# raulmur/ORB_SLAM2

Hardware: NVIDIA H100
Metric: stereo frames/sec (ORB extract L+R + ComputeStereoMatches, KITTI-shaped 1242x375 @2000 kpts) (higher is better)
Workload: dtype u8

## Files before the change

### orb_slam2_b200/csrc/borb_host.cu

```cuda
#include <cmath>
#include <cstdarg>
#include <cstdio>
#include <algorithm>
#include <cstdlib>
#include <cstring>

#include "borb_internal.h"

namespace borb {

static thread_local std::string tl_error;
void set_error(const char* fmt, ...) {
    char buf[512];
    va_list ap;
    va_start(ap, fmt);
    vsnprintf(buf, sizeof(buf), fmt, ap);
    va_end(ap);
    tl_error = buf;
}

bool allow_max_smem(const void* func) {
    static std::mutex mu;
    static std::vector<std::pair<const void*, int>> done;
    int dev = 0;
// ... 123 lines not shown
        v.hCell = (int)std::ceil(height / v.nRows);
        v.pitch = align_up(v.w + 8, 128);
        v.pyr_off = pyr_off;
        pyr_off += (unsigned)v.pitch * v.h;
        v.cellsPerBlk = FAST_TILE_W / v.wCell > 0 ? FAST_TILE_W / v.wCell : 1;
        v.blkCols = (v.nCols + v.cellsPerBlk - 1) / v.cellsPerBlk;
        v.blkBase = blk;
        blk += v.blkCols * v.nRows;
        v.cand_off = cand_off;
        v.cand_cap = v.nCols * v.nRows * ((v.wCell + 1) / 2) * ((v.hCell + 1) / 2);
        cand_off += (unsigned)align_up(v.cand_cap, 32);
        v.quota = e->per_level[l];
        v.nIni = (int)std::round(width / height);
        if (v.nIni < 1) { set_error("level %d aspect ratio gives zero quadtree roots (reference divides by zero)", l); return BORB_ERR_UNSUPPORTED; }
        v.hX = width / v.nIni;
        v.node_cap = (v.quota > 4 * v.nIni ? v.quota : 4 * v.nIni) + 3;
        v.node_cap = align_up(v.node_cap + 1, 4);
        v.sel_off = sel_off;
        sel_off += v.node_cap;
        v.scale = e->scale[l];
        v.inv_scale = e->inv_scale[l];
        v.patch_size = (float)(int)(PATCH * e->scale[l]);
        g.blur_base[l] = btile;
        btile += ((v.w + BLUR_TILE_W - 1) / BLUR_TILE_W) * ((v.h + BLUR_TILE_H - 1) / BLUR_TILE_H);
        if (l > 0) {
            const int wpad = (v.w + 8 + 3) & ~3;
            v.xtab_off = (unsigned)(tabs.size() / 4);
            resize_table(g.lv[l - 1].w, v.w, true, wpad - v.w, tabs);
            v.ytab_off = (unsigned)(tabs.size() / 4);
            resize_table(g.lv[l - 1].h, v.h, false, 0, tabs);
            v.xwin_off = (unsigned)(tabs.size() / 4);
            std::vector<int16_t> win;
            v.x_windowed = resize_window_table(tabs, (size_t)v.xtab_off * 4, wpad, win) ? 1 : 0;
            tabs.insert(tabs.end(), win.begin(), win.end());
        }
        if (quadtree_smem_bytes(v.node_cap) > 200 * 1024) {
            set_error("per-level quota %d exceeds the quadtree kernel's shared-memory envelope", v.quota);
            return BORB_ERR_UNSUPPORTED;
        }
    }
    g.blur_base[L] = btile;
    g.blur_tiles = btile;
    g.fast_blocks = blk;
    g.pyr_image_stride = (unsigned)align_up((int)pyr_off, g.lv[0].pitch);
    g.cand_image_stride = cand_off;
    g.sel_image_stride = sel_off;
    if (sel_off >= 65536) { set_error("keypoint capacity %d exceeds 65535", sel_off); return BORB_ERR_UNSUPPORTED; }
// ... 75 lines not shown
    cudaEventRecord(e->ev[(size_t)e->ev_slot * 9 + i], e->stream);
    e->ev_mask[e->ev_slot] |= 1u << i;
}
void drain_timing(borb_extractor* e) {
    const int R = borb_extractor::EV_RING;
    for (int k = e->ev_pending - 1; k >= 0; k--) {
        const int slot = ((e->ev_slot - k) % R + R) % R;
        const unsigned m = e->ev_mask[slot];
        for (int i = 0; i < 8; i++) {
            float ms = 0.f;
            if (m & (1u << i)) {
                int j = i + 1;
                while (j < 9 && !(m & (1u << j))) j++;
                if (j < 9 && cudaEventElapsedTime(&ms, e->ev[(size_t)slot * 9 + i], e->ev[(size_t)slot * 9 + j]) != cudaSuccess) { ms = 0.f; cudaGetLastError(); }
            }
            e->stage_ms[i] = ms;
            e->stage_sum_ms[i] += ms;
        }
        e->stage_steps++;
    }
    e->ev_pending = 0;
}

borb_status enqueue_extract(borb_extractor* e, int n) {
    const Geometry& g = e->geom;
    Workspace& ws = e->ws;
    cudaStream_t s = e->stream;
    BORB_CUDA(cudaMemsetAsync(ws.cand_cnt, 0, (size_t)n * g.nlevels * sizeof(int), s));
    mark(e, 1);
    e->launches += launch_pyramid(g, ws, n, s);
    mark(e, 2);
    e->launches += launch_fast(g, ws, n, s);
    mark(e, 3);
    e->launches += launch_quadtree(g, ws, n, s);
    mark(e, 4);
    e->launches += launch_blur(g, ws, n, s);
    mark(e, 5);
    e->launches += launch_describe(g, ws, n, s);
    mark(e, 6);
    BORB_CUDA(cudaGetLastError());
    e->last_n_images = n;
    e->last_stereo_pairs = 0;
    return BORB_OK;
}

borb_status rectified_size(borb_extractor* e, int w, int h, int* gw, int* gh) {
    if (!e->d_map[0][0]) return BORB_OK;
    if (w != e->map_src_w || h != e->map_src_h) {
        set_error("rectification maps were built for %dx%d raw frames, got %dx%d", e->map_src_w, e->map_src_h, w, h);
        return BORB_ERR_INVALID_ARG;
    }
    *gw = e->map_dst_w; *gh = e->map_dst_h;
    return BORB_OK;
}

borb_status upload_slots(borb_extractor* e, const uint8_t* const* slots, int n, int w, int h, int stride, bool stereo_pairs = false) {
    const Geometry& g = e->geom;
    const int ch = e->in_channels;
    if (stride < w * ch) { set_error("stride %d smaller than a row of %d %d-channel pixels", stride, w, ch); return BORB_ERR_INVALID_ARG; }
    const size_t img_bytes = (size_t)stride * h;
    bool contiguous = n > 1 || ch > 1 || e->d_map[0][0] != nullptr;
    for (int k = 0; k < n; k++) {
        if (!slots[k]) { set_error("image %d is NULL", k); return BORB_ERR_INVALID_ARG; }
        if (slots[k] != slots[0] + (size_t)k * img_bytes) contiguous = false;
    }
    auto need_stage = [&](size_t need) -> borb_status {
        if (e->ws.stage_bytes < need) {
            BORB_CUDA(cudaStreamSynchronize(e->stream));
            cudaFree(e->ws.stage);
            e->ws.stage = nullptr; e->ws.stage_bytes = 0;
            BORB_CUDA(cudaMalloc(&e->ws.stage, need));
            e->ws.stage_bytes = need;
        }
        return BORB_OK;
    };
    if (e->d_map[0][0]) {
        if (ch != 1) { set_error("rectification maps apply to CV_8UC1 frames"); return BORB_ERR_UNSUPPORTED; }
        const size_t src_img = contiguous ? img_bytes : (size_t)w * h;
        const int src_stride = contiguous ? stride : w;
        borb_status st = need_stage(src_img * n);
        if (st != BORB_OK) return st;
        if (contiguous) BORB_CUDA(cudaMemcpyAsync(e->ws.stage, slots[0], src_img * n, cudaMemcpyHostToDevice, e->stream));
        else
            for (int k = 0; k < n; k++)
                BORB_CUDA(cudaMemcpy2DAsync(e->ws.stage + (size_t)k * src_img, w, slots[k], stride, w, h, cudaMemcpyHostToDevice, e->stream));
        e->launches += launch_repack_remap(g, e->ws, e->ws.stage, src_stride, src_img, w, h, e->d_map[0][0], e->d_map[0][1],
                                           stereo_pairs ? e->d_map[1][0] : nullptr, stereo_pairs ? e->d_map[1][1] : nullptr, n, e->stream);
        return BORB_OK;
    }
    if (contiguous) {
        const size_t need = img_bytes * n;
        borb_status st = need_stage(need);
        if (st != BORB_OK) return st;
        BORB_CUDA(cudaMemcpyAsync(e->ws.stage, slots[0], need, cudaMemcpyHostToDevice, e->stream));
        if (ch == 1) e->launches += launch_repack(g, e->ws, e->ws.stage, stride, img_bytes, n, e->stream);
        else e->launches += launch_repack_color(g, e->ws, e->ws.stage, stride, img_bytes, ch, e->in_rgb, n, e->stream);
        return BORB_OK;
    }
    if (ch > 1) {
        const size_t row = (size_t)w * ch;
        borb_status st = need_stage(row * h * n);
        if (st != BORB_OK) return st;
        for (int k = 0; k < n; k++)
            BORB_CUDA(cudaMemcpy2DAsync(e->ws.stage + (size_t)k * row * h, row, slots[k], stride, row, h, cudaMemcpyHostToDevice, e->stream));
        e->launches += launch_repack_color(g, e->ws, e->ws.stage, (int)row, row * h, ch, e->in_rgb, n, e->stream);
        return BORB_OK;
    }
    for (int k = 0; k < n; k++) {
        uint8_t* dst = e->ws.pyr + (size_t)k * g.pyr_image_stride + g.lv[0].pyr_off;
        BORB_CUDA(cudaMemcpy2DAsync(dst, g.lv[0].pitch, slots[k], stride, w, h, cudaMemcpyHostToDevice, e->stream));
    }
    return BORB_OK;
}

borb_status upload_device(borb_extractor* e, const uint8_t* d_gray, int n, int w, int h, size_t pitch, size_t image_stride) {
    const Geometry& g = e->geom;
    cudaMemcpy3DParms p = {};
    p.srcPtr = make_cudaPitchedPtr((void*)d_gray, pitch, w, image_stride / pitch);
    p.dstPtr = make_cudaPitchedPtr(e->ws.pyr + g.lv[0].pyr_off, g.lv[0].pitch, w, g.pyr_image_stride / g.lv[0].pitch);
    if (image_stride % pitch == 0 && g.pyr_image_stride % g.lv[0].pitch == 0) {
        p.extent = make_cudaExtent(w, h, n);
        p.kind = cudaMemcpyDeviceToDevice;
        BORB_CUDA(cudaMemcpy3DAsync(&p, e->stream));
    } else {
        for (int i = 0; i < n; i++)
            BORB_CUDA(cudaMemcpy2DAsync(e->ws.pyr + (size_t)i * g.pyr_image_stride + g.lv[0].pyr_off, g.lv[0].pitch,
                                        d_gray + (size_t)i * image_stride, pitch, w, h, cudaMemcpyDeviceToDevice, e->stream));
    }
    return BORB_OK;
}

borb_status download_kps(borb_extractor* e, int first, int count, int step, borb_keypoint* kps, uint8_t* desc, int cap, int* n_out) {
    const Geometry& g = e->geom;
    const int m = cap < g.sel_image_stride ? cap : g.sel_image_stride;
    cudaStream_t s = e->stream;
    if (kps && m > 0)
        BORB_CUDA(cudaMemcpy2DAsync(kps, (size_t)cap * sizeof(borb_keypoint), e->ws.kps + (size_t)first * g.sel_image_stride,
                                    (size_t)step * g.sel_image_stride * sizeof(borb_keypoint), (size_t)m * sizeof(borb_keypoint),
                                    count, cudaMemcpyDeviceToHost, s));
    if (desc && m > 0)
        BORB_CUDA(cudaMemcpy2DAsync(desc, (size_t)cap * 32, e->ws.desc + (size_t)first * g.sel_image_stride * 32,
                                    (size_t)step * g.sel_image_stride * 32, (size_t)m * 32, count, cudaMemcpyDeviceToHost, s));
    if (n_out)
        BORB_CUDA(cudaMemcpy2DAsync(n_out, sizeof(int), e->ws.nkp + first, (size_t)step * sizeof(int), sizeof(int), count,
                                    cudaMemcpyDeviceToHost, s));
    return BORB_OK;
}

borb_status check_args(borb_extractor* e, int n, int w, int h) {
    if (!e) { set_error("null handle"); return BORB_ERR_INVALID_ARG; }
// ... 157 lines not shown
borb_status borb_extractor_reserve(borb_extractor* e, int width, int height, int max_images) {
    if (!e || max_images < 1) return BORB_ERR_INVALID_ARG;
    return ensure(e, width, height, max_images);
}

borb_status borb_sync(borb_extractor* e) {
    if (!e) return BORB_ERR_INVALID_ARG;
    BORB_CUDA(cudaSetDevice(e->device));
    BORB_CUDA(cudaStreamSynchronize(e->stream));
    return finish_timing(e);
}

borb_status borb_extract_batch_enqueue(borb_extractor* e, const uint8_t* const* gray, int n, int w, int h, int stride,
                                       borb_keypoint* kps, uint8_t* desc, int cap, int* n_out) {
    borb_status st = check_args(e, n, w, h);
    if (st != BORB_OK) return st;
    if (n == 0) return BORB_OK;
    if (!gray || cap < 0 || stride < w) { set_error("bad arguments"); return BORB_ERR_INVALID_ARG; }
    int gw = w, gh = h;
    if ((st = rectified_size(e, w, h, &gw, &gh)) != BORB_OK) return st;
    if ((st = ensure(e, gw, gh, n)) != BORB_OK) return st;
    begin_step(e);
    mark(e, 0);
    if ((st = upload_slots(e, gray, n, w, h, stride)) != BORB_OK) return st;
    if ((st = enqueue_extract(e, n)) != BORB_OK) return st;
    mark(e, 7);
    st = download_kps(e, 0, n, 1, kps, desc, cap, n_out);
    mark(e, 8);
    return st;
}

borb_status borb_extract_batch(borb_extractor* e, const uint8_t* const* gray, int n, int w, int h, int stride,
                               borb_keypoint* kps, uint8_t* desc, int cap, int* n_out) {
    if (!n_out) { set_error("n_out is required"); return BORB_ERR_INVALID_ARG; }
    borb_status st = borb_extract_batch_enqueue(e, gray, n, w, h, stride, kps, desc, cap, n_out);
    if (st != BORB_OK) return st;
    if (n == 0) return BORB_OK;
    if ((st = borb_sync(e)) != BORB_OK) return st;
    for (int i = 0; i < n; i++)
        if (n_out[i] > cap) { set_error("image %d produced %d keypoints, capacity %d", i, n_out[i], cap); return BORB_ERR_CAPACITY; }
    return BORB_OK;
}

borb_status borb_extract(borb_extractor* e, const uint8_t* gray, int w, int h, int stride, borb_keypoint* kps, uint8_t* desc,
                         int cap, int* n_out) {
    if (!n_out) { set_error("n_out is required"); return BORB_ERR_INVALID_ARG; }
    *n_out = 0;
    if (!gray || w == 0 || h == 0) return BORB_OK;
    const uint8_t* one[1] = {gray};
    return borb_extract_batch(e, one, 1, w, h, stride, kps, desc, cap, n_out);
}

borb_status borb_extract_batch_device(borb_extractor* e, const uint8_t* d_gray, int n, int w, int h, size_t pitch,
                                      size_t image_stride, borb_keypoint* kps, uint8_t* desc, int cap, int* n_out) {
    borb_status st = check_args(e, n, w, h);
    if (st != BORB_OK) return st;
    if (n == 0) return BORB_OK;
    if (!d_gray || pitch < (size_t)w) { set_error("bad arguments"); return BORB_ERR_INVALID_ARG; }
    if ((st = ensure(e, w, h, n)) != BORB_OK) return st;
    begin_step(e);
    mark(e, 0);
    if ((st = upload_device(e, d_gray, n, w, h, pitch, image_stride)) != BORB_OK) return st;
    if ((st = enqueue_extract(e, n)) != BORB_OK) return st;
    mark(e, 7);
    if ((st = download_kps(e, 0, n, 1, kps, desc, cap, n_out)) != BORB_OK) return st;
    mark(e, 8);
    return borb_sync(e);
}

borb_status borb_extractor_set_rectify_maps(borb_extractor* e, int which, const float* map_x, const float* map_y, int src_w, int src_h,
                                            int dst_w, int dst_h) {
    if (!e || which < 0 || which > 1) { set_error("bad arguments"); return BORB_ERR_INVALID_ARG; }
    BORB_CUDA(cudaSetDevice(e->device));
    BORB_CUDA(cudaStreamSynchronize(e->stream));
    if (!map_x || !map_y) {
        for (int s2 = which; s2 < 2; s2++)
            for (int c = 0; c < 2; c++) { cudaFree(e->d_map[s2][c]); e->d_map[s2][c] = nullptr; }
        return BORB_OK;
    }
    if (src_w <= 0 || src_h <= 0 || dst_w <= 0 || dst_h <= 0) { set_error("bad map geometry"); return BORB_ERR_INVALID_ARG; }
    if (which == 1 && (!e->d_map[0][0] || src_w != e->map_src_w || src_h != e->map_src_h || dst_w != e->map_dst_w || dst_h != e->map_dst_h)) {
        set_error("install the left maps (set 0) first; both sets share one geometry"); return BORB_ERR_STATE;
    }
    const size_t bytes = (size_t)dst_w * dst_h * sizeof(float);
    const float* src[2] = {map_x, map_y};
    for (int c = 0; c < 2; c++) {
// ... 138 lines not shown
    BORB_CUDA(cudaSetDevice(left->device));
    BORB_CUDA(cudaStreamSynchronize(right->stream));
    begin_step(left);
    borb_status st = enqueue_stereo(left, right, 1, nullptr, nullptr, bf, b);
    if (st != BORB_OK) return st;
    if ((st = download_stereo(left, 1, u_right, depth, cap)) != BORB_OK) return st;
    mark(left, 8);
    return borb_sync(left);
}

borb_status borb_stereo_frames_enqueue(borb_extractor* e, const uint8_t* const* left, const uint8_t* const* right, int n_pairs,
                                       int w, int h, int stride, float bf, float b, borb_keypoint* kps_left, uint8_t* desc_left,
                                       int* n_left, borb_keypoint* kps_right, uint8_t* desc_right, int* n_right, float* u_right,
                                       float* depth, int cap) {
    borb_status st = check_args(e, n_pairs, w, h);
    if (st != BORB_OK) return st;
    if (n_pairs == 0) return BORB_OK;
    if (!left || !right || stride < w || !(b > 0.f)) { set_error("bad arguments"); return BORB_ERR_INVALID_ARG; }
    int gw = w, gh = h;
    if ((st = rectified_size(e, w, h, &gw, &gh)) != BORB_OK) return st;
    if ((st = ensure(e, gw, gh, 2 * n_pairs)) != BORB_OK) return st;
    begin_step(e);
    mark(e, 0);
    {
        std::vector<const uint8_t*> slots(2 * (size_t)n_pairs);
        for (int p = 0; p < n_pairs; p++) { slots[2 * p] = left[p]; slots[2 * p + 1] = right[p]; }
        if ((st = upload_slots(e, slots.data(), 2 * n_pairs, w, h, stride, true)) != BORB_OK) return st;
    }
    if ((st = enqueue_extract(e, 2 * n_pairs)) != BORB_OK) return st;
    if ((st = enqueue_stereo(e, e, n_pairs, nullptr, nullptr, bf, b)) != BORB_OK) return st;
    if ((st = download_kps(e, 0, n_pairs, 2, kps_left, desc_left, cap, n_left)) != BORB_OK) return st;
    if ((st = download_kps(e, 1, n_pairs, 2, kps_right, desc_right, cap, n_right)) != BORB_OK) return st;
    if ((st = download_stereo(e, n_pairs, u_right, depth, cap)) != BORB_OK) return st;
    mark(e, 8);
    return BORB_OK;
}

borb_status borb_stereo_frames(borb_extractor* e, const uint8_t* const* left, const uint8_t* const* right, int n_pairs, int w,
                               int h, int stride, float bf, float b, borb_keypoint* kps_left, uint8_t* desc_left, int* n_left,
                               borb_keypoint* kps_right, uint8_t* desc_right, int* n_right, float* u_right, float* depth, int cap) {
    borb_status st = borb_stereo_frames_enqueue(e, left, right, n_pairs, w, h, stride, bf, b, kps_left, desc_left, n_left,
                                                kps_right, desc_right, n_right, u_right, depth, cap);
    if (st != BORB_OK || n_pairs == 0) return st;
    if ((st = borb_sync(e)) != BORB_OK) return st;
    for (int p = 0; p < n_pairs; p++)
        if ((n_left && n_left[p] > cap) || (n_right && n_right[p] > cap)) { set_error("pair %d exceeds capacity %d", p, cap); return BORB_ERR_CAPACITY; }
    return BORB_OK;
}

borb_status borb_stereo_frames_device_enqueue(borb_extractor* e, const uint8_t* d_gray, int n_pairs, int w, int h, size_t pitch,
                                              size_t image_stride, float bf, float b, int* n_left, int* n_right, float* u_right,
                                              float* depth, int cap) {
    borb_status st = check_args(e, n_pairs, w, h);
    if (st != BORB_OK) return st;
    if (n_pairs == 0) return BORB_OK;
    if (!d_gray || pitch < (size_t)w || !(b > 0.f)) { set_error("bad arguments"); return BORB_ERR_INVALID_ARG; }
    if ((st = ensure(e, w, h, 2 * n_pairs)) != BORB_OK) return st;
    begin_step(e);
    mark(e, 0);
    if ((st = upload_device(e, d_gray, 2 * n_pairs, w, h, pitch, image_stride)) != BORB_OK) return st;
    if ((st = enqueue_extract(e, 2 * n_pairs)) != BORB_OK) return st;
    if ((st = enqueue_stereo(e, e, n_pairs, nullptr, nullptr, bf, b)) != BORB_OK) return st;
    if ((st = download_kps(e, 0, n_pairs, 2, nullptr, nullptr, cap, n_left)) != BORB_OK) return st;
    if ((st = download_kps(e, 1, n_pairs, 2, nullptr, nullptr, cap, n_right)) != BORB_OK) return st;
    if ((st = download_stereo(e, n_pairs, u_right, depth, cap)) != BORB_OK) return st;
    mark(e, 8);
    return BORB_OK;
}

borb_status borb_stereo_frames_device(borb_extractor* e, const uint8_t* d_gray, int n_pairs, int w, int h, size_t pitch,
                                      size_t image_stride, float bf, float b, int* n_left, int* n_right, float* u_right,
                                      float* depth, int cap) {
    borb_status st = borb_stereo_frames_device_enqueue(e, d_gray, n_pairs, w, h, pitch, image_stride, bf, b, n_left, n_right,
                                                       u_right, depth, cap);
    if (st != BORB_OK || n_pairs == 0) return st;
    return borb_sync(e);
}

borb_status borb_stereo_frames_results(borb_extractor* e, int n_pairs, borb_keypoint* kps_left, uint8_t* desc_left, int* n_left,
                                       borb_keypoint* kps_right, uint8_t* desc_right, int* n_right, float* u_right, float* depth,
                                       int cap) {
    if (!e || n_pairs < 0 || cap < 0) { set_error("bad arguments"); return BORB_ERR_INVALID_ARG; }
    if (n_pairs == 0) return BORB_OK;
    if (!e->have_geom || n_pairs > e->last_stereo_pairs) {
// ... 18 lines not shown
```

### orb_slam2_b200/csrc/borb_internal.h

```cpp
#pragma once
#include <cuda_runtime.h>
#include <stdint.h>

#include <mutex>
#include <string>
#include <vector>

#include "../../include/borb.h"

namespace borb {

constexpr int EDGE = 19;
constexpr int PATCH = 31;
constexpr int HALF_PATCH = 15;
constexpr int MIN_BORDER = 16;
constexpr int TH_HIGH = 100;
constexpr int TH_LOW = 50;
constexpr int BLUR_TILE_W = 120;
constexpr int BLUR_TILE_H = 64;
constexpr int FAST_TILE_W = 124;

__host__ __device__ inline uint32_t pack_xys(int x, int y, int s) { return (uint32_t)x | ((uint32_t)y << 12) | ((uint32_t)s << 24); }
__host__ __device__ inline int xys_x(uint32_t v) { return (int)(v & 0xFFFu); }
__host__ __device__ inline int xys_y(uint32_t v) { return (int)((v >> 12) & 0xFFFu); }
__host__ __device__ inline int xys_s(uint32_t v) { return (int)(v >> 24); }

struct LevelGeom {
    int w, h;
    int pitch;
    unsigned pyr_off;
    int nCols, nRows, wCell, hCell;
    int cellsPerBlk;
    int blkCols;
    int blkBase;
    unsigned cand_off;
    int cand_cap;
    int quota;
    int nIni;
    float hX;
    int node_cap;
    int sel_off;
// ... 41 lines not shown
    void* st_recs = nullptr;
    uint8_t* stage = nullptr;
    size_t stage_bytes = 0;
    void* fast_tmaps = nullptr;
    void* fast_tiles = nullptr;
    int fast_n_tiles = 0;
};

void set_error(const char* fmt, ...);
bool allow_max_smem(const void* func);
#define BORB_CUDA(call)                                                                             \
    do {                                                                                            \
        cudaError_t _e = (call);                                                                    \
        if (_e != cudaSuccess) {                                                                    \
            borb::set_error("%s failed: %s (%s:%d)", #call, cudaGetErrorString(_e), __FILE__, __LINE__); \
            return (_e == cudaErrorNoDevice || _e == cudaErrorInsufficientDriver) ? BORB_ERR_NO_DEVICE : BORB_ERR_CUDA; \
        }                                                                                           \
    } while (0)

int launch_repack_remap(const Geometry& g, const Workspace& ws, const uint8_t* stage, int src_stride, size_t src_image_bytes, int src_w,
                        int src_h, const float* mx0, const float* my0, const float* mx1, const float* my1, int n_images, cudaStream_t s);
int launch_repack_color(const Geometry& g, const Workspace& ws, const uint8_t* stage, int src_stride, size_t src_image_bytes, int channels,
                        int rgb, int n_images, cudaStream_t s);
int launch_repack(const Geometry& g, const Workspace& ws, const uint8_t* stage, int src_stride, size_t src_image_bytes,
                  int n_images, cudaStream_t s);
int launch_pyramid(const Geometry& g, const Workspace& ws, int n_images, cudaStream_t s);
int launch_fast(const Geometry& g, const Workspace& ws, int n_images, cudaStream_t s);
int launch_quadtree(const Geometry& g, const Workspace& ws, int n_images, cudaStream_t s);
int launch_blur(const Geometry& g, const Workspace& ws, int n_images, cudaStream_t s);
int launch_describe(const Geometry& g, const Workspace& ws, int n_images, cudaStream_t s);

struct StereoView {
    const uint8_t* pyr;
    const borb_keypoint* kps;
    const uint8_t* desc;
    const int* nkp;
    unsigned pyr_image_stride;
    int kp_image_stride;
};
int launch_stereo(const Geometry& g, const StereoView& L, const StereoView& R, const int* d_pair_idx, int n_pairs,
                  float bf, float b, float* d_u_right, float* d_depth, int* d_sad, int out_stride, int* d_bins, void* d_recs,
                  cudaStream_t s);
int stereo_rec_stride(const Geometry& g);
size_t stereo_bins_bytes_per_pair();
size_t stereo_rec_bytes();
size_t quadtree_smem_bytes(int node_cap);
borb_status build_fast_tmaps(const Geometry& g, const Workspace& ws, void* out_tmaps);
borb_status build_fast_tiles(const Geometry& g, Workspace& ws);
size_t fast_tmaps_bytes();
// ... 34 lines not shown
```

### orb_slam2_b200/csrc/k_blur.cu

```cuda
#include "borb_internal.h"

namespace borb {

namespace {
constexpr int BT_R = 16;
constexpr int BT_WARPS = BLUR_TILE_H / BT_R;

__device__ __forceinline__ int reflect101(int p, int len) {
    if (p < 0) p = -p;
    if (p >= len) p = 2 * len - 2 - p;
    return min(max(p, 0), len - 1);
}
}

__global__ void __launch_bounds__(32 * BT_WARPS) blur_kernel(const __grid_constant__ Geometry g, const uint8_t* __restrict__ pyr,
                                                             uint8_t* __restrict__ blur) {
    const int img = blockIdx.y;
    int l = 0;
    while (l + 1 < g.nlevels && (int)blockIdx.x >= g.blur_base[l + 1]) l++;
    const LevelGeom& L = g.lv[l];
    const int local = blockIdx.x - g.blur_base[l];
    const int tilesX = (L.w + BLUR_TILE_W - 1) / BLUR_TILE_W;
    const int ty = local / tilesX, tx = local - ty * tilesX;
    const int lane = threadIdx.x & 31, wrp = threadIdx.x >> 5;
    const int x = tx * BLUR_TILE_W + 4 * (lane - 1);
    const int yb = ty * BLUR_TILE_H + wrp * BT_R;
    if (yb >= L.h) return;
    const uint8_t* src = pyr + (size_t)img * g.pyr_image_stride + L.pyr_off;
    uint8_t* dst = blur + (size_t)img * g.pyr_image_stride + L.pyr_off;
    const int W = L.w, H = L.h, pitch = L.pitch;
    const bool left_edge = (x == 0);
    const bool loads = x >= 0 && x < pitch;
    const bool stores = lane >= 1 && lane <= 30 && x < W;
    const unsigned WLO = 18u | (34u << 8) | (48u << 16) | (56u << 24);
    const unsigned WHI = 48u | (34u << 8) | (18u << 16);

    uint32_t own[BT_R + 6];
    if (yb >= 3 && yb + BT_R + 2 < H) {
        const uint8_t* p = src + (size_t)(yb - 3) * pitch + x;
#pragma unroll
        for (int step = 0; step < BT_R + 6; step++, p += pitch) own[step] = loads ? *reinterpret_cast<const uint32_t*>(p) : 0u;
    } else {
#pragma unroll
        for (int step = 0; step < BT_R + 6; step++)
            own[step] = loads ? *reinterpret_cast<const uint32_t*>(src + (unsigned)(reflect101(yb + step - 3, H) * pitch) + x) : 0u;
    }

    uint32_t pk[6][4];
    uint32_t hprev[4] = {0, 0, 0, 0};
#pragma unroll
    for (int step = 0; step < BT_R + 6; step++) {
        const uint32_t W1 = own[step];
        uint32_t W0 = __shfl_up_sync(0xFFFFFFFFu, W1, 1);
        const uint32_t W2 = __shfl_down_sync(0xFFFFFFFFu, W1, 1);
        if (left_edge) W0 = __byte_perm(W1, W2, 0x1234);
        uint32_t h[4];
        h[0] = __dp4a(__byte_perm(W0, W1, 0x4321), WLO, __dp4a(__byte_perm(W1, W2, 0x4321), WHI, 0u));
        h[1] = __dp4a(__byte_perm(W0, W1, 0x5432), WLO, __dp4a(__byte_perm(W1, W2, 0x5432), WHI, 0u));
        h[2] = __dp4a(__byte_perm(W0, W1, 0x6543), WLO, __dp4a(__byte_perm(W1, W2, 0x6543), WHI, 0u));
        h[3] = __dp4a(W1, WLO, __dp4a(W2, WHI, 0u));
        if (step >= 1) {
#pragma unroll
            for (int i = 0; i < 4; i++) pk[(step - 1) % 6][i] = __byte_perm(hprev[i], h[i], 0x5410);
        }
        if (step >= 6) {
            const int yout = yb + step - 6;
            if (yout < H && stores) {
                uint32_t s[4];
#pragma unroll
                for (int i = 0; i < 4; i++) {
                    uint32_t acc = h[i] * 18u + 32768u;
                    acc = __dp2a_lo(pk[(step - 2) % 6][i], 48u | (34u << 8), acc);
                    acc = __dp2a_lo(pk[(step - 4) % 6][i], 48u | (56u << 8), acc);
                    s[i] = __dp2a_lo(pk[(step - 6) % 6][i], 18u | (34u << 8), acc);
                }
                const uint32_t out = __byte_perm(__byte_perm(s[0], s[1], 0x0062), __byte_perm(s[2], s[3], 0x0062), 0x5410);
                *reinterpret_cast<uint32_t*>(dst + (size_t)yout * pitch + x) = out;
            }
        }
#pragma unroll
        for (int i = 0; i < 4; i++) hprev[i] = h[i];
    }
}

int launch_blur(const Geometry& g, const Workspace& ws, int n_images, cudaStream_t s) {
    dim3 grid(g.blur_tiles, n_images);
    blur_kernel<<<grid, 32 * BT_WARPS, 0, s>>>(g, ws.pyr, ws.blur);
    return 1;
}

}
```

### orb_slam2_b200/csrc/k_pyramid.cu

```cuda
#include "borb_internal.h"

namespace borb {

template <int ROWS>
__global__ void __launch_bounds__(256, 6) pyr_resize_kernel(const uint8_t* __restrict__ pyr, uint8_t* __restrict__ pyr_out,
                                                         const int16_t* __restrict__ tabs, LevelGeom src, LevelGeom dst,
                                                         unsigned image_stride) {
    const int img = blockIdx.z;
    const int dyb = (blockIdx.y * 8 + threadIdx.y) * ROWS;
    const int dx0 = (blockIdx.x * 32 + threadIdx.x) * 4;
    const int wpad = (dst.w + 8 + 3) & ~3;
    if (dyb >= dst.h || dx0 >= wpad) return;
    const uint8_t* S = pyr + (size_t)img * image_stride + src.pyr_off;
    uint8_t* D = pyr_out + (size_t)img * image_stride + dst.pyr_off;
    const uint4* xt = reinterpret_cast<const uint4*>(tabs + ((size_t)dst.xwin_off + dx0) * 4);
    const uint2* yt = reinterpret_cast<const uint2*>(tabs + (size_t)dst.ytab_off * 4);
    const uint4 e01 = xt[0], e23 = xt[1];
    const uint32_t wts[4] = {e01.x, e01.z, e23.x, e23.z};
    const uint32_t ctl[4] = {e01.y, e01.w, e23.y, e23.w};
    const int base = (int)(ctl[0] & 0xFFFF);
    uint32_t ra[ROWS][3], rc[ROWS][3];
    uint32_t B0[ROWS], B1[ROWS];
#pragma unroll
    for (int r = 0; r < ROWS; r++) {
        const int dy = min(dyb + r, dst.h - 1);
// ... 25 lines not shown
}

__global__ void __launch_bounds__(256) pyr_resize_generic_kernel(const uint8_t* __restrict__ pyr, uint8_t* __restrict__ pyr_out,
                                                                 const int16_t* __restrict__ tabs, LevelGeom src, LevelGeom dst,
                                                                 unsigned image_stride) {
    const int img = blockIdx.z;
    const int dy = blockIdx.y * 8 + threadIdx.y;
    const int dx = blockIdx.x * 32 + threadIdx.x;
    const int wpad = (dst.w + 8 + 3) & ~3;
    if (dy >= dst.h || dx >= wpad) return;
    const uint8_t* S = pyr + (size_t)img * image_stride + src.pyr_off;
    uint8_t* D = pyr_out + (size_t)img * image_stride + dst.pyr_off;
    const short4 xe = reinterpret_cast<const short4*>(tabs)[(size_t)dst.xtab_off + dx];
    const short4 ye = reinterpret_cast<const short4*>(tabs)[(size_t)dst.ytab_off + dy];
    const int sy0 = min(max((int)ye.x, 0), src.h - 1), sy1 = min(max((int)ye.x + 1, 0), src.h - 1);
    const uint8_t* R0 = S + (size_t)sy0 * src.pitch;
    const uint8_t* R1 = S + (size_t)sy1 * src.pitch;
    const int sx = xe.x;
    const int r0 = R0[sx] * xe.y + R0[sx + 1] * xe.z;
    const int r1 = R1[sx] * xe.y + R1[sx + 1] * xe.z;
    D[(size_t)dy * dst.pitch + dx] = (uint8_t)((((ye.y * (r0 >> 4)) >> 16) + ((ye.z * (r1 >> 4)) >> 16) + 2) >> 2);
}

__global__ void __launch_bounds__(256) repack_kernel(const uint8_t* __restrict__ stage, int src_stride, size_t src_image_bytes,
                                                     uint8_t* __restrict__ pyr, LevelGeom l0, unsigned image_stride) {
    const int img = blockIdx.z, y = blockIdx.y;
    const int x0 = (blockIdx.x * 256 + threadIdx.x) * 4;
    if (x0 >= l0.w) return;
    const uint8_t* S = stage + (size_t)img * src_image_bytes + (size_t)y * src_stride + x0;
    uint32_t v = 0;
#pragma unroll
    for (int i = 0; i < 4; i++)
        if (x0 + i < l0.w) v |= (uint32_t)S[i] << (8 * i);
    *reinterpret_cast<uint32_t*>(pyr + (size_t)img * image_stride + l0.pyr_off + (size_t)y * l0.pitch + x0) = v;
}

__global__ void __launch_bounds__(256) repack_color_kernel(const uint8_t* __restrict__ stage, int src_stride, size_t src_image_bytes,
                                                           int channels, int rgb, uint8_t* __restrict__ pyr, LevelGeom l0,
                                                           unsigned image_stride) {
    const int img = blockIdx.z, y = blockIdx.y;
    const int x0 = (blockIdx.x * 256 + threadIdx.x) * 4;
    if (x0 >= l0.w) return;
    const uint8_t* S = stage + (size_t)img * src_image_bytes + (size_t)y * src_stride + (size_t)x0 * channels;
    const int cr = rgb ? 9798 : 3735, cb = rgb ? 3735 : 9798;
    uint32_t v = 0;
#pragma unroll
    for (int i = 0; i < 4; i++)
        if (x0 + i < l0.w) {
            const uint8_t* px = S + i * channels;
            const int yv = (px[0] * cr + px[1] * 19235 + px[2] * cb + 16384) >> 15;
            v |= (uint32_t)yv << (8 * i);
        }
    *reinterpret_cast<uint32_t*>(pyr + (size_t)img * image_stride + l0.pyr_off + (size_t)y * l0.pitch + x0) = v;
}

__global__ void __launch_bounds__(256) repack_remap_kernel(const uint8_t* __restrict__ stage, int src_stride, size_t src_image_bytes,
                                                           int src_w, int src_h, const float* __restrict__ mx0,
                                                           const float* __restrict__ my0, const float* __restrict__ mx1,
                                                           const float* __restrict__ my1, uint8_t* __restrict__ pyr, LevelGeom l0,
// ... 3 lines not shown
    if (x0 >= l0.w) return;
    const bool second = (img & 1) && mx1 != nullptr;
    const float* MX = second ? mx1 : mx0;
    const float* MY = second ? my1 : my0;
    const uint8_t* S = stage + (size_t)img * src_image_bytes;
    uint32_t v = 0;
#pragma unroll
    for (int i = 0; i < 4; i++)
        if (x0 + i < l0.w) {
            const size_t o = (size_t)y * l0.w + x0 + i;
            const int sx = __float2int_rn(__fmul_rn(MX[o], 32.f)), sy = __float2int_rn(__fmul_rn(MY[o], 32.f));
            const int ix = max(-32768, min(32767, sx >> 5)), iy = max(-32768, min(32767, sy >> 5));
            const int fx = sx & 31, fy = sy & 31;
            auto tap = [&](int yy, int xx) -> int {
                return (xx >= 0 && xx < src_w && yy >= 0 && yy < src_h) ? (int)S[(size_t)yy * src_stride + xx] : 0;
            };
            const int w00 = (32 - fx) * (32 - fy) * 32, w01 = fx * (32 - fy) * 32, w10 = (32 - fx) * fy * 32, w11 = fx * fy * 32;
            const int r = (tap(iy, ix) * w00 + tap(iy, ix + 1) * w01 + tap(iy + 1, ix) * w10 + tap(iy + 1, ix + 1) * w11 + 16384) >> 15;
            v |= (uint32_t)r << (8 * i);
        }
    *reinterpret_cast<uint32_t*>(pyr + (size_t)img * image_stride + l0.pyr_off + (size_t)y * l0.pitch + x0) = v;
}

__global__ void __launch_bounds__(256) pad_level0_kernel(uint8_t* __restrict__ pyr, LevelGeom l0, unsigned image_stride) {
    const int y = blockIdx.x * 256 + threadIdx.x, img = blockIdx.y;
    if (y >= l0.h) return;
    uint8_t* row = pyr + (size_t)img * image_stride + l0.pyr_off + (size_t)y * l0.pitch;
#pragma unroll
    for (int k = 0; k < 8; k++) row[l0.w + k] = row[max(l0.w - 2 - k, 0)];
}

int launch_repack(const Geometry& g, const Workspace& ws, const uint8_t* stage, int src_stride, size_t src_image_bytes,
                  int n_images, cudaStream_t s) {
    dim3 grid((g.lv[0].w + 1023) / 1024, g.lv[0].h, n_images);
    repack_kernel<<<grid, 256, 0, s>>>(stage, src_stride, src_image_bytes, ws.pyr, g.lv[0], g.pyr_image_stride);
    return 1;
}

constexpr int PYR_ROWS = 2;

int launch_repack_remap(const Geometry& g, const Workspace& ws, const uint8_t* stage, int src_stride, size_t src_image_bytes, int src_w,
                        int src_h, const float* mx0, const float* my0, const float* mx1, const float* my1, int n_images, cudaStream_t s) {
    dim3 grid((g.lv[0].w + 1023) / 1024, g.lv[0].h, n_images);
    repack_remap_kernel<<<grid, 256, 0, s>>>(stage, src_stride, src_image_bytes, src_w, src_h, mx0, my0, mx1, my1, ws.pyr, g.lv[0],
                                             g.pyr_image_stride);
    return 1;
}

int launch_repack_color(const Geometry& g, const Workspace& ws, const uint8_t* stage, int src_stride, size_t src_image_bytes, int channels,
                        int rgb, int n_images, cudaStream_t s) {
    dim3 grid((g.lv[0].w + 1023) / 1024, g.lv[0].h, n_images);
    repack_color_kernel<<<grid, 256, 0, s>>>(stage, src_stride, src_image_bytes, channels, rgb, ws.pyr, g.lv[0], g.pyr_image_stride);
    return 1;
}

int launch_pyramid(const Geometry& g, const Workspace& ws, int n_images, cudaStream_t s) {
    int launches = 0;
    pad_level0_kernel<<<dim3((g.lv[0].h + 255) / 256, n_images), 256, 0, s>>>(ws.pyr, g.lv[0], g.pyr_image_stride);
    launches++;
    for (int l = 1; l < g.nlevels; l++) {
        const LevelGeom& d = g.lv[l];
        dim3 block(32, 8);
        if (d.x_windowed) {
            dim3 grid((d.w + 8 + 127) / 128, (d.h + 8 * PYR_ROWS - 1) / (8 * PYR_ROWS), n_images);
            pyr_resize_kernel<PYR_ROWS><<<grid, block, 0, s>>>(ws.pyr, ws.pyr, ws.tabs, g.lv[l - 1], d, g.pyr_image_stride);
        } else {
            dim3 grid((d.w + 8 + 3 + 31) / 32, (d.h + 7) / 8, n_images);
            pyr_resize_generic_kernel<<<grid, block, 0, s>>>(ws.pyr, ws.pyr, ws.tabs, g.lv[l - 1], d, g.pyr_image_stride);
        }
        launches++;
    }
    return launches;
}

}
```

Before: 39530.

## Fuse level-0 repack, border padding and Gaussian blur into one producer kernel

Level 0 of the pyramid is now produced by a single kernel that reads the staged or device input, writes it into the pyramid with reflected right-edge padding, and computes the blurred level-0 image in the same pass. The separate repack, pad and device-to-device copy steps are removed, and the blur kernel now skips level 0. The blur kernel tile width becomes 128, with edge lanes doing extra halo loads instead of sacrificing two lanes per warp to the halo. This cuts launches and a full read/write round trip of the largest level, at the cost of extra complexity and an in-place mode for data already in the pyramid.

```diff
diff --git a/orb_slam2_b200/csrc/borb_host.cu b/orb_slam2_b200/csrc/borb_host.cu
--- a/orb_slam2_b200/csrc/borb_host.cu
+++ b/orb_slam2_b200/csrc/borb_host.cu
@@ -169,7 +169,7 @@
         v.inv_scale = e->inv_scale[l];
         v.patch_size = (float)(int)(PATCH * e->scale[l]);
         g.blur_base[l] = btile;
-        btile += ((v.w + BLUR_TILE_W - 1) / BLUR_TILE_W) * ((v.h + BLUR_TILE_H - 1) / BLUR_TILE_H);
+        if (l > 0) btile += ((v.w + BLUR_TILE_W - 1) / BLUR_TILE_W) * ((v.h + BLUR_TILE_H - 1) / BLUR_TILE_H);
         if (l > 0) {
             const int wpad = (v.w + 8 + 3) & ~3;
             v.xtab_off = (unsigned)(tabs.size() / 4);
@@ -291,13 +291,13 @@
     e->ev_pending = 0;
 }
 
-borb_status enqueue_extract(borb_extractor* e, int n) {
+borb_status enqueue_extract(borb_extractor* e, int n, const Level0Source& l0) {
     const Geometry& g = e->geom;
     Workspace& ws = e->ws;
     cudaStream_t s = e->stream;
     BORB_CUDA(cudaMemsetAsync(ws.cand_cnt, 0, (size_t)n * g.nlevels * sizeof(int), s));
     mark(e, 1);
-    e->launches += launch_pyramid(g, ws, n, s);
+    e->launches += launch_pyramid(g, ws, l0, n, s);
     mark(e, 2);
     e->launches += launch_fast(g, ws, n, s);
     mark(e, 3);
@@ -323,7 +323,8 @@
     return BORB_OK;
 }
 
-borb_status upload_slots(borb_extractor* e, const uint8_t* const* slots, int n, int w, int h, int stride, bool stereo_pairs = false) {
+borb_status upload_slots(borb_extractor* e, const uint8_t* const* slots, int n, int w, int h, int stride, Level0Source* l0,
+                         bool stereo_pairs = false) {
     const Geometry& g = e->geom;
     const int ch = e->in_channels;
     if (stride < w * ch) { set_error("stride %d smaller than a row of %d %d-channel pixels", stride, w, ch); return BORB_ERR_INVALID_ARG; }
@@ -362,7 +363,7 @@
         borb_status st = need_stage(need);
         if (st != BORB_OK) return st;
         BORB_CUDA(cudaMemcpyAsync(e->ws.stage, slots[0], need, cudaMemcpyHostToDevice, e->stream));
-        if (ch == 1) e->launches += launch_repack(g, e->ws, e->ws.stage, stride, img_bytes, n, e->stream);
+        if (ch == 1) *l0 = Level0Source{e->ws.stage, (size_t)stride, img_bytes};
         else e->launches += launch_repack_color(g, e->ws, e->ws.stage, stride, img_bytes, ch, e->in_rgb, n, e->stream);
         return BORB_OK;
     }
@@ -378,23 +379,6 @@
     for (int k = 0; k < n; k++) {
         uint8_t* dst = e->ws.pyr + (size_t)k * g.pyr_image_stride + g.lv[0].pyr_off;
         BORB_CUDA(cudaMemcpy2DAsync(dst, g.lv[0].pitch, slots[k], stride, w, h, cudaMemcpyHostToDevice, e->stream));
-    }
-    return BORB_OK;
-}
-
-borb_status upload_device(borb_extractor* e, const uint8_t* d_gray, int n, int w, int h, size_t pitch, size_t image_stride) {
-    const Geometry& g = e->geom;
-    cudaMemcpy3DParms p = {};
-    p.srcPtr = make_cudaPitchedPtr((void*)d_gray, pitch, w, image_stride / pitch);
-    p.dstPtr = make_cudaPitchedPtr(e->ws.pyr + g.lv[0].pyr_off, g.lv[0].pitch, w, g.pyr_image_stride / g.lv[0].pitch);
-    if (image_stride % pitch == 0 && g.pyr_image_stride % g.lv[0].pitch == 0) {
-        p.extent = make_cudaExtent(w, h, n);
-        p.kind = cudaMemcpyDeviceToDevice;
-        BORB_CUDA(cudaMemcpy3DAsync(&p, e->stream));
-    } else {
-        for (int i = 0; i < n; i++)
-            BORB_CUDA(cudaMemcpy2DAsync(e->ws.pyr + (size_t)i * g.pyr_image_stride + g.lv[0].pyr_off, g.lv[0].pitch,
-                                        d_gray + (size_t)i * image_stride, pitch, w, h, cudaMemcpyDeviceToDevice, e->stream));
     }
     return BORB_OK;
 }
@@ -598,8 +582,9 @@
     if ((st = ensure(e, gw, gh, n)) != BORB_OK) return st;
     begin_step(e);
     mark(e, 0);
-    if ((st = upload_slots(e, gray, n, w, h, stride)) != BORB_OK) return st;
-    if ((st = enqueue_extract(e, n)) != BORB_OK) return st;
+    Level0Source l0;
+    if ((st = upload_slots(e, gray, n, w, h, stride, &l0)) != BORB_OK) return st;
+    if ((st = enqueue_extract(e, n, l0)) != BORB_OK) return st;
     mark(e, 7);
     st = download_kps(e, 0, n, 1, kps, desc, cap, n_out);
     mark(e, 8);
@@ -636,8 +621,7 @@
     if ((st = ensure(e, w, h, n)) != BORB_OK) return st;
     begin_step(e);
     mark(e, 0);
-    if ((st = upload_device(e, d_gray, n, w, h, pitch, image_stride)) != BORB_OK) return st;
-    if ((st = enqueue_extract(e, n)) != BORB_OK) return st;
+    if ((st = enqueue_extract(e, n, Level0Source{d_gray, pitch, image_stride})) != BORB_OK) return st;
     mark(e, 7);
     if ((st = download_kps(e, 0, n, 1, kps, desc, cap, n_out)) != BORB_OK) return st;
     mark(e, 8);
@@ -822,12 +806,13 @@
     if ((st = ensure(e, gw, gh, 2 * n_pairs)) != BORB_OK) return st;
     begin_step(e);
     mark(e, 0);
+    Level0Source l0;
     {
         std::vector<const uint8_t*> slots(2 * (size_t)n_pairs);
         for (int p = 0; p < n_pairs; p++) { slots[2 * p] = left[p]; slots[2 * p + 1] = right[p]; }
-        if ((st = upload_slots(e, slots.data(), 2 * n_pairs, w, h, stride, true)) != BORB_OK) return st;
-    }
-    if ((st = enqueue_extract(e, 2 * n_pairs)) != BORB_OK) return st;
+        if ((st = upload_slots(e, slots.data(), 2 * n_pairs, w, h, stride, &l0, true)) != BORB_OK) return st;
+    }
+    if ((st = enqueue_extract(e, 2 * n_pairs, l0)) != BORB_OK) return st;
     if ((st = enqueue_stereo(e, e, n_pairs, nullptr, nullptr, bf, b)) != BORB_OK) return st;
     if ((st = download_kps(e, 0, n_pairs, 2, kps_left, desc_left, cap, n_left)) != BORB_OK) return st;
     if ((st = download_kps(e, 1, n_pairs, 2, kps_right, desc_right, cap, n_right)) != BORB_OK) return st;
@@ -858,8 +843,7 @@
     if ((st = ensure(e, w, h, 2 * n_pairs)) != BORB_OK) return st;
     begin_step(e);
     mark(e, 0);
-    if ((st = upload_device(e, d_gray, 2 * n_pairs, w, h, pitch, image_stride)) != BORB_OK) return st;
-    if ((st = enqueue_extract(e, 2 * n_pairs)) != BORB_OK) return st;
+    if ((st = enqueue_extract(e, 2 * n_pairs, Level0Source{d_gray, pitch, image_stride})) != BORB_OK) return st;
     if ((st = enqueue_stereo(e, e, n_pairs, nullptr, nullptr, bf, b)) != BORB_OK) return st;
     if ((st = download_kps(e, 0, n_pairs, 2, nullptr, nullptr, cap, n_left)) != BORB_OK) return st;
     if ((st = download_kps(e, 1, n_pairs, 2, nullptr, nullptr, cap, n_right)) != BORB_OK) return st;
diff --git a/orb_slam2_b200/csrc/borb_internal.h b/orb_slam2_b200/csrc/borb_internal.h
--- a/orb_slam2_b200/csrc/borb_internal.h
+++ b/orb_slam2_b200/csrc/borb_internal.h
@@ -16,7 +16,7 @@
 constexpr int MIN_BORDER = 16;
 constexpr int TH_HIGH = 100;
 constexpr int TH_LOW = 50;
-constexpr int BLUR_TILE_W = 120;
+constexpr int BLUR_TILE_W = 128;
 constexpr int BLUR_TILE_H = 64;
 constexpr int FAST_TILE_W = 124;
 
@@ -104,9 +104,11 @@
                         int src_h, const float* mx0, const float* my0, const float* mx1, const float* my1, int n_images, cudaStream_t s);
 int launch_repack_color(const Geometry& g, const Workspace& ws, const uint8_t* stage, int src_stride, size_t src_image_bytes, int channels,
                         int rgb, int n_images, cudaStream_t s);
-int launch_repack(const Geometry& g, const Workspace& ws, const uint8_t* stage, int src_stride, size_t src_image_bytes,
-                  int n_images, cudaStream_t s);
-int launch_pyramid(const Geometry& g, const Workspace& ws, int n_images, cudaStream_t s);
+struct Level0Source {
+    const uint8_t* ptr = nullptr;
+    size_t pitch = 0, image_stride = 0;
+};
+int launch_pyramid(const Geometry& g, const Workspace& ws, const Level0Source& l0, int n_images, cudaStream_t s);
 int launch_fast(const Geometry& g, const Workspace& ws, int n_images, cudaStream_t s);
 int launch_quadtree(const Geometry& g, const Workspace& ws, int n_images, cudaStream_t s);
 int launch_blur(const Geometry& g, const Workspace& ws, int n_images, cudaStream_t s);
diff --git a/orb_slam2_b200/csrc/k_blur.cu b/orb_slam2_b200/csrc/k_blur.cu
--- a/orb_slam2_b200/csrc/k_blur.cu
+++ b/orb_slam2_b200/csrc/k_blur.cu
@@ -23,27 +23,35 @@
     const int tilesX = (L.w + BLUR_TILE_W - 1) / BLUR_TILE_W;
     const int ty = local / tilesX, tx = local - ty * tilesX;
     const int lane = threadIdx.x & 31, wrp = threadIdx.x >> 5;
-    const int x = tx * BLUR_TILE_W + 4 * (lane - 1);
+    const int x = tx * BLUR_TILE_W + 4 * lane;
+    const int xe = lane == 0 ? x - 4 : x + 4;
     const int yb = ty * BLUR_TILE_H + wrp * BT_R;
     if (yb >= L.h) return;
     const uint8_t* src = pyr + (size_t)img * g.pyr_image_stride + L.pyr_off;
     uint8_t* dst = blur + (size_t)img * g.pyr_image_stride + L.pyr_off;
     const int W = L.w, H = L.h, pitch = L.pitch;
     const bool left_edge = (x == 0);
-    const bool loads = x >= 0 && x < pitch;
-    const bool stores = lane >= 1 && lane <= 30 && x < W;
+    const bool loads = x < pitch;
+    const bool eloads = (lane == 0 || lane == 31) && xe >= 0 && xe < pitch;
+    const bool stores = x < W;
     const unsigned WLO = 18u | (34u << 8) | (48u << 16) | (56u << 24);
     const unsigned WHI = 48u | (34u << 8) | (18u << 16);
 
-    uint32_t own[BT_R + 6];
+    uint32_t own[BT_R + 6], ext[BT_R + 6];
     if (yb >= 3 && yb + BT_R + 2 < H) {
-        const uint8_t* p = src + (size_t)(yb - 3) * pitch + x;
+        const uint8_t* p = src + (size_t)(yb - 3) * pitch;
 #pragma unroll
-        for (int step = 0; step < BT_R + 6; step++, p += pitch) own[step] = loads ? *reinterpret_cast<const uint32_t*>(p) : 0u;
+        for (int step = 0; step < BT_R + 6; step++, p += pitch) {
+            own[step] = loads ? *reinterpret_cast<const uint32_t*>(p + x) : 0u;
+            ext[step] = eloads ? *reinterpret_cast<const uint32_t*>(p + xe) : 0u;
+        }
     } else {
 #pragma unroll
-        for (int step = 0; step < BT_R + 6; step++)
-            own[step] = loads ? *reinterpret_cast<const uint32_t*>(src + (unsigned)(reflect101(yb + step - 3, H) * pitch) + x) : 0u;
+        for (int step = 0; step < BT_R + 6; step++) {
+            const uint8_t* p = src + (unsigned)(reflect101(yb + step - 3, H) * pitch);
+            own[step] = loads ? *reinterpret_cast<const uint32_t*>(p + x) : 0u;
+            ext[step] = eloads ? *reinterpret_cast<const uint32_t*>(p + xe) : 0u;
+        }
     }
 
     uint32_t pk[6][4];
@@ -52,7 +60,9 @@
     for (int step = 0; step < BT_R + 6; step++) {
         const uint32_t W1 = own[step];
         uint32_t W0 = __shfl_up_sync(0xFFFFFFFFu, W1, 1);
-        const uint32_t W2 = __shfl_down_sync(0xFFFFFFFFu, W1, 1);
+        uint32_t W2 = __shfl_down_sync(0xFFFFFFFFu, W1, 1);
+        if (lane == 0) W0 = ext[step];
+        if (lane == 31) W2 = ext[step];
         if (left_edge) W0 = __byte_perm(W1, W2, 0x1234);
         uint32_t h[4];
         h[0] = __dp4a(__byte_perm(W0, W1, 0x4321), WLO, __dp4a(__byte_perm(W1, W2, 0x4321), WHI, 0u));
@@ -84,6 +94,7 @@
 }
 
 int launch_blur(const Geometry& g, const Workspace& ws, int n_images, cudaStream_t s) {
+    if (g.blur_tiles == 0) return 0;
     dim3 grid(g.blur_tiles, n_images);
     blur_kernel<<<grid, 32 * BT_WARPS, 0, s>>>(g, ws.pyr, ws.blur);
     return 1;
diff --git a/orb_slam2_b200/csrc/k_pyramid.cu b/orb_slam2_b200/csrc/k_pyramid.cu
--- a/orb_slam2_b200/csrc/k_pyramid.cu
+++ b/orb_slam2_b200/csrc/k_pyramid.cu
@@ -1,6 +1,120 @@
 #include "borb_internal.h"
 
 namespace borb {
+
+namespace {
+constexpr int L0_TILE_W = 120;
+constexpr int PROD_R = 16;
+constexpr int PROD_WARPS = BLUR_TILE_H / PROD_R;
+
+enum { PROD_COPY = 1, PROD_IN_PLACE = 2 };
+
+__device__ __forceinline__ int reflect101(int p, int len) {
+    if (p < 0) p = -p;
+    if (p >= len) p = 2 * len - 2 - p;
+    return min(max(p, 0), len - 1);
+}
+
+__device__ __forceinline__ uint32_t row_word(const uint8_t* row, int x, bool inside) {
+    const uintptr_t a = reinterpret_cast<uintptr_t>(row + x);
+    const uint32_t* p = reinterpret_cast<const uint32_t*>(a & ~(uintptr_t)3);
+    const unsigned sh = (unsigned)(a & 3) * 8;
+    const uint32_t w0 = inside ? p[0] : 0u;
+    const uint32_t w1 = inside && sh ? p[1] : 0u;
+    return __funnelshift_r(w0, w1, sh);
+}
+__device__ __forceinline__ uint32_t row_edge_word(const uint8_t* row, int x, int W) {
+    uint32_t v = 0;
+#pragma unroll
+    for (int i = 0; i < 4; i++) {
+        const int xx = x + i;
+        v |= (uint32_t)row[xx < W ? xx : max(2 * W - 2 - xx, 0)] << (8 * i);
+    }
+    return v;
+}
+}
+
+template <int MODE>
+__global__ void __launch_bounds__(32 * PROD_WARPS) level0_kernel(uint8_t* pyr, uint8_t* __restrict__ blur, LevelGeom dst, unsigned image_stride,
+                                                                 const uint8_t* in, size_t in_pitch, size_t in_image_stride) {
+    const int img = blockIdx.z;
+    const int lane = threadIdx.x & 31, wrp = threadIdx.x >> 5;
+    const int x = blockIdx.x * L0_TILE_W + 4 * (lane - 1);
+    const int yb = (blockIdx.y * PROD_WARPS + wrp) * PROD_R;
+    const int W = dst.w, H = dst.h, pitch = dst.pitch;
+    if (yb >= H) return;
+    const int wpad = (W + 8 + 3) & ~3;
+    const bool live = x >= 0 && x < wpad;
+    const bool owner = live && lane >= 1 && lane <= 30;
+    uint8_t* P = pyr + (size_t)img * image_stride + dst.pyr_off;
+    uint8_t* B = blur + (size_t)img * image_stride + dst.pyr_off;
+
+    uint32_t own[PROD_R + 6];
+    {
+        const uint8_t* I = in + (size_t)img * in_image_stride;
+        const bool inside = x >= 0 && x + 4 <= W;
+#pragma unroll
+        for (int step = 0; step < PROD_R + 6; step++) own[step] = row_word(I + (size_t)reflect101(yb + step - 3, H) * in_pitch, x, inside);
+        if (live && !inside) {
+#pragma unroll
+            for (int step = 0; step < PROD_R + 6; step++)
+                own[step] = row_edge_word(I + (size_t)reflect101(yb + step - 3, H) * in_pitch, x, W);
+        }
+    }
+#pragma unroll
+    for (int step = 3; step < PROD_R + 3; step++) {
+        const int y = yb + step - 3;
+        if (y >= H || !owner) continue;
+        uint8_t* row = P + (size_t)y * pitch;
+        if (MODE != PROD_IN_PLACE) {
+            *reinterpret_cast<uint32_t*>(row + x) = own[step];
+        } else if (x + 4 > W) {
+#pragma unroll
+            for (int i = 0; i < 4; i++)
+                if (x + i >= W && x + i < W + 8) row[x + i] = (uint8_t)(own[step] >> (8 * i));
+        }
+    }
+
+    const bool left_edge = (x == 0);
+    const bool stores = lane >= 1 && lane <= 30 && x < W;
+    const unsigned WLO = 18u | (34u << 8) | (48u << 16) | (56u << 24);
+    const unsigned WHI = 48u | (34u << 8) | (18u << 16);
+    uint32_t pk[6][4];
+    uint32_t hprev[4] = {0, 0, 0, 0};
+#pragma unroll
+    for (int step = 0; step < PROD_R + 6; step++) {
+        const uint32_t W1 = own[step];
+        uint32_t W0 = __shfl_up_sync(0xFFFFFFFFu, W1, 1);
+        const uint32_t W2 = __shfl_down_sync(0xFFFFFFFFu, W1, 1);
+        if (left_edge) W0 = __byte_perm(W1, W2, 0x1234);
+        uint32_t h[4];
+        h[0] = __dp4a(__byte_perm(W0, W1, 0x4321), WLO, __dp4a(__byte_perm(W1, W2, 0x4321), WHI, 0u));
+        h[1] = __dp4a(__byte_perm(W0, W1, 0x5432), WLO, __dp4a(__byte_perm(W1, W2, 0x5432), WHI, 0u));
+        h[2] = __dp4a(__byte_perm(W0, W1, 0x6543), WLO, __dp4a(__byte_perm(W1, W2, 0x6543), WHI, 0u));
+        h[3] = __dp4a(W1, WLO, __dp4a(W2, WHI, 0u));
+        if (step >= 1) {
+#pragma unroll
+            for (int i = 0; i < 4; i++) pk[(step - 1) % 6][i] = __byte_perm(hprev[i], h[i], 0x5410);
+        }
+        if (step >= 6) {
+            const int yout = yb + step - 6;
+            if (yout < H && stores) {
+                uint32_t s[4];
+#pragma unroll
+                for (int i = 0; i < 4; i++) {
+                    uint32_t acc = h[i] * 18u + 32768u;
+                    acc = __dp2a_lo(pk[(step - 2) % 6][i], 48u | (34u << 8), acc);
+                    acc = __dp2a_lo(pk[(step - 4) % 6][i], 48u | (56u << 8), acc);
+                    s[i] = __dp2a_lo(pk[(step - 6) % 6][i], 18u | (34u << 8), acc);
+                }
+                const uint32_t out = __byte_perm(__byte_perm(s[0], s[1], 0x0062), __byte_perm(s[2], s[3], 0x0062), 0x5410);
+                *reinterpret_cast<uint32_t*>(B + (size_t)yout * pitch + x) = out;
+            }
+        }
+#pragma unroll
+        for (int i = 0; i < 4; i++) hprev[i] = h[i];
+    }
+}
 
 template <int ROWS>
 __global__ void __launch_bounds__(256, 6) pyr_resize_kernel(const uint8_t* __restrict__ pyr, uint8_t* __restrict__ pyr_out,
@@ -72,19 +186,6 @@
     D[(size_t)dy * dst.pitch + dx] = (uint8_t)((((ye.y * (r0 >> 4)) >> 16) + ((ye.z * (r1 >> 4)) >> 16) + 2) >> 2);
 }
 
-__global__ void __launch_bounds__(256) repack_kernel(const uint8_t* __restrict__ stage, int src_stride, size_t src_image_bytes,
-                                                     uint8_t* __restrict__ pyr, LevelGeom l0, unsigned image_stride) {
-    const int img = blockIdx.z, y = blockIdx.y;
-    const int x0 = (blockIdx.x * 256 + threadIdx.x) * 4;
-    if (x0 >= l0.w) return;
-    const uint8_t* S = stage + (size_t)img * src_image_bytes + (size_t)y * src_stride + x0;
-    uint32_t v = 0;
-#pragma unroll
-    for (int i = 0; i < 4; i++)
-        if (x0 + i < l0.w) v |= (uint32_t)S[i] << (8 * i);
-    *reinterpret_cast<uint32_t*>(pyr + (size_t)img * image_stride + l0.pyr_off + (size_t)y * l0.pitch + x0) = v;
-}
-
 __global__ void __launch_bounds__(256) repack_color_kernel(const uint8_t* __restrict__ stage, int src_stride, size_t src_image_bytes,
                                                            int channels, int rgb, uint8_t* __restrict__ pyr, LevelGeom l0,
                                                            unsigned image_stride) {
@@ -134,21 +235,6 @@
     *reinterpret_cast<uint32_t*>(pyr + (size_t)img * image_stride + l0.pyr_off + (size_t)y * l0.pitch + x0) = v;
 }
 
-__global__ void __launch_bounds__(256) pad_level0_kernel(uint8_t* __restrict__ pyr, LevelGeom l0, unsigned image_stride) {
-    const int y = blockIdx.x * 256 + threadIdx.x, img = blockIdx.y;
-    if (y >= l0.h) return;
-    uint8_t* row = pyr + (size_t)img * image_stride + l0.pyr_off + (size_t)y * l0.pitch;
-#pragma unroll
-    for (int k = 0; k < 8; k++) row[l0.w + k] = row[max(l0.w - 2 - k, 0)];
-}
-
-int launch_repack(const Geometry& g, const Workspace& ws, const uint8_t* stage, int src_stride, size_t src_image_bytes,
-                  int n_images, cudaStream_t s) {
-    dim3 grid((g.lv[0].w + 1023) / 1024, g.lv[0].h, n_images);
-    repack_kernel<<<grid, 256, 0, s>>>(stage, src_stride, src_image_bytes, ws.pyr, g.lv[0], g.pyr_image_stride);
-    return 1;
-}
-
 constexpr int PYR_ROWS = 2;
 
 int launch_repack_remap(const Geometry& g, const Workspace& ws, const uint8_t* stage, int src_stride, size_t src_image_bytes, int src_w,
@@ -166,10 +252,15 @@
     return 1;
 }
 
-int launch_pyramid(const Geometry& g, const Workspace& ws, int n_images, cudaStream_t s) {
-    int launches = 0;
-    pad_level0_kernel<<<dim3((g.lv[0].h + 255) / 256, n_images), 256, 0, s>>>(ws.pyr, g.lv[0], g.pyr_image_stride);
-    launches++;
+int launch_pyramid(const Geometry& g, const Workspace& ws, const Level0Source& l0, int n_images, cudaStream_t s) {
+    const LevelGeom& d0 = g.lv[0];
+    const dim3 grid0((((d0.w + 8 + 3) & ~3) + L0_TILE_W - 1) / L0_TILE_W, (d0.h + BLUR_TILE_H - 1) / BLUR_TILE_H, n_images);
+    if (l0.ptr)
+        level0_kernel<PROD_COPY><<<grid0, 32 * PROD_WARPS, 0, s>>>(ws.pyr, ws.blur, d0, g.pyr_image_stride, l0.ptr, l0.pitch, l0.image_stride);
+    else
+        level0_kernel<PROD_IN_PLACE><<<grid0, 32 * PROD_WARPS, 0, s>>>(ws.pyr, ws.blur, d0, g.pyr_image_stride, ws.pyr + d0.pyr_off, d0.pitch,
+                                                                       g.pyr_image_stride);
+    int launches = 1;
     for (int l = 1; l < g.nlevels; l++) {
         const LevelGeom& d = g.lv[l];
         dim3 block(32, 8);
```

Measured after the change: 40180, median of 6. 1.7% higher.
